# louislung/DAE_RNN_News_Recommendation

Hardware: NVIDIA H100
Metric: articles/sec (higher is better)
Workload: dtype f32

## Files before the change

### dae_rnn_news_recommendation_b200/_cabi.py

```python
import ctypes
import ctypes as C
import os
from pathlib import Path

_PKG = Path(__file__).resolve().parent
LIB_PATH = Path(os.environ.get('DAE_SM100_LIB', _PKG / 'libdae_sm100.so'))

ACT = {'none': 0, 'sigmoid': 1, 'tanh': 2}
LOSS = {'cross_entropy': 0, 'mean_squared': 1, 'cosine_proximity': 2}
STRATEGY = {'none': 0, 'batch_all': 1, 'batch_hard': 2, 'explicit': 3}
OPT = {'gradient_descent': 0, 'ada_grad': 1, 'momentum': 2, 'adam': 3}
STAT = {'cost': 0, 'ae_loss': 1, 'triplet_loss': 2, 'fraction': 3, 'num': 4, 'sum_w': 5, 'n_valid': 6, 'sum_lw': 7,
        'triplet_sum': 8, 'n_active': 9}
STAT_SLOTS = 16
MAX_TRIPLET_BATCH = 32768
MAX_BLOCKED_BATCH = 262144


def act_code(name):
    return ACT.get(name, 0)


p, i32, i64, f32, u64, sz = C.c_void_p, C.c_int32, C.c_int64, C.c_float, C.c_uint64, C.c_size_t

_SIGNATURES = {
    'dae_version': (C.c_int, []),
    'dae_last_error': (C.c_int, [C.c_char_p, sz]),
    'dae_batch_prepare': (C.c_int, [p, i64, p, i32, p, i32, p, p, p, p, p, p, p]),
    'dae_batch_prepare_next': (C.c_int, [p, i64, i64, p, i32, p, i32, p, p, p, p, p, p, p]),
    'dae_batch_prepare_blocked': (C.c_int, [p, i64, p, i32, p, i32, p, p, p, p, p, p, p]),
    'dae_batch_prepare_next_blocked': (C.c_int, [p, i64, i64, p, i32, p, i32, p, p, p, p, p, p, p]),
    'dae_batch_commit': (C.c_int, [i32, p, p, p, p, p, p, p, p, p, p, p, p, p]),
    'dae_batch_prepare_explicit': (C.c_int, [p, i64, p, i32, i64, p, p, p]),
    'dae_step_advance': (C.c_int, [p, i64, p]),
    'dae_encode_csr_fwd': (C.c_int, [p, p, p, p, i32, i32, i32, f32, p, p, i32, p, i64, p, p, p, i64, p]),
    'dae_encode_csr_fwd_hot': (C.c_int, [p, p, p, i32, i32, i32, f32, p, p, i32, p, i64, p, p, i32, i32, p]),
    'dae_col_scan': (C.c_int, [p, i32, p, p, p]),
    'dae_encode_csr_bwd_gather': (C.c_int, [p, p, p, p, i32, i32, i32, f32, p, p, i32, p, p, i64, p, p, i32, p, p, p, p, p, p, p]),
    'dae_encode_csr_bwd': (C.c_int, [p, p, p, p, i32, i32, i32, f32, p, p, i32, p, p, i64, p, p, i32, p]),
    'dae_sgemm': (C.c_int, [i32, i32, i32, f32, p, i64, i64, p, i64, i64, f32, p, i64, p]),
    'dae_split_bf16': (C.c_int, [p, i32, i32, i64, p, p, i64, i32, f32, p]),
    'dae_sym_split_bf16': (C.c_int, [p, i32, i64, f32, p, p, i64, p]),
    'dae_gemm_bf16x3': (C.c_int, [i32, i32, i32, f32, p, p, i64, i32, p, p, i64, i32, p, i64, i32, i32, p, i32, i32, p]),
    'dae_gemm_config': (C.c_int, [i32, i32]),
    'dae_decode_prepare': (C.c_int, [i32, i32, p, p, p, p, p, p]),
    'dae_decode_fused_bf16x3': (C.c_int, [i32, i32, i32, p, p, i64, p, p, i64, p, p, p, p, p, i32, i32, p, p, p, p, i64, p, p, i32, p]),
    'dae_reduce_parts': (C.c_int, [p, i32, i32, p, p]),
    'dae_decode_loss_bwd': (C.c_int, [p, p, p, p, i32, i32, p, i32, i32, p, p, p, i64, p, p]),
    'dae_colsum': (C.c_int, [p, i32, i32, i64, p, p]),
    'dae_triplet_batch_all': (C.c_int, [p, i64, i32, p, p, p, i64, p, i32, p, p, i64, p]),
    'dae_triplet_config': (C.c_int, [i32]),
    'dae_gemm_sym_bf16x3': (C.c_int, [i32, i32, f32, p, p, i64, p, p, i64, p, i64, i32, p]),
    'dae_triplet_batch_hard': (C.c_int, [p, i64, i32, p, p, i64, p, p, p]),
    'dae_triplet_batch_all_rows': (C.c_int, [p, i64, i32, i32, i32, p, p, p, i64, p, i32, p, p, i64, p]),
    'dae_triplet_batch_hard_rows': (C.c_int, [p, i64, i32, i32, i32, p, p, i64, p, p, p]),
    'dae_triplet_batch_hard_finish': (C.c_int, [p, i32, p, p, i32, i64, p]),
    'dae_triplet_explicit': (C.c_int, [p, p, p, i32, i32, i64, f32, p, p, p, p, p]),
    'dae_step_finalize': (C.c_int, [p, p, i32, p, i32, i32, f32, p, p, p, p]),
    'dae_optimizer_step': (C.c_int, [p, p, p, p, i64, i32, f32, f32, f32, i32, p, p, p, i32, i32, i64, p]),
    'dae_rownorm_split_bf16': (C.c_int, [p, i32, i32, i64, i32, p, p, i64, p, i64, p]),
    'dae_row_argmax': (C.c_int, [p, i32, i32, i64, i64, i32, p, p, p]),
    'dae_similarity_topk_bf16x3': (C.c_int, [i32, i32, i32, p, p, i64, p, p, i64, i32, i64, i32, i32, p, i64, p, p, p]),
    'dae_similarity_topk_workspace': (C.c_int, [i32, i32, i32, i32, p]),
    'dae_csr_similarity_topk': (C.c_int, [p, p, p, i32, i64, i32, p, p, p, i32, i64, i32, i32, i64, i32, i32, p, i64, p, p, p]),
    'dae_csr_similarity_topk_workspace': (C.c_int, [i32, i32, i64, i32, i32, i32, p]),
    'dae_similarity_topk_excl_bf16x3': (C.c_int, [i32, i32, i32, p, p, i64, p, p, i64, i32, i64, i32, i32, p, i64, p, p, p, p, i64, p]),
    'dae_csr_similarity_topk_excl': (C.c_int, [p, p, p, i32, i64, i32, p, p, p, i32, i64, i32, i32, i64, i32, i32, p, i64, p, p, p, p,
                                               i64, p]),
    'dae_similarity_topk_groups_bf16x3': (C.c_int, [i32, i32, i32, p, p, i64, p, p, i64, i32, i64, i32, i32, p, i64, p, p, p, p, i64, p,
                                                    p]),
    'dae_csr_similarity_topk_groups': (C.c_int, [p, p, p, i32, i64, i32, p, p, p, i32, i64, i32, i32, i64, i32, i32, p, i64, p, p, p, p,
# ... 121 lines not shown
```

### dae_rnn_news_recommendation_b200/csrc/encode.cu

```cuda
#include <algorithm>
#include <cstdlib>
#include <cuda_bf16.h>
#include "common.cuh"

namespace dae {

template <int VW> struct Vec;
template <> struct Vec<4> { using T = float4; };
template <> struct Vec<2> { using T = float2; };
template <> struct Vec<1> { using T = float; };

template <int VW>
__device__ __forceinline__ void ldg_vec(const float* p, float (&out)[VW]) {
  if constexpr (VW == 4) { const float4 v = __ldg(reinterpret_cast<const float4*>(p)); out[0] = v.x; out[1] = v.y; out[2] = v.z; out[3] = v.w; }
  else if constexpr (VW == 2) { const float2 v = __ldg(reinterpret_cast<const float2*>(p)); out[0] = v.x; out[1] = v.y; }
  else { out[0] = __ldg(p); }
}

constexpr int kEncThreads = 128;

template <int NT = 128>
__device__ __forceinline__ int stage_row_chunk(const int32_t* __restrict__ indices, const float* __restrict__ values,
                                               int64_t base, int64_t p1, float in_scale, int* s_col, float* s_val,
                                               int* s_wcnt) {
// ... 260 lines not shown
  if (tid == 0) s_carry = 0;
  __syncthreads();
  for (int base = 0; base < F; base += kChunkElems) {
    const int n = min(kChunkElems, F - base);
    for (int i = tid; i < kChunkElems; i += 1024) s[i] = (i < n) ? col_count[base + i] : 0;
    __syncthreads();
    int v[kPer], sum = 0;
#pragma unroll
    for (int j = 0; j < kPer; ++j) { v[j] = s[tid * kPer + j]; sum += v[j]; }
    int incl = sum;
#pragma unroll
    for (int o = 1; o < 32; o <<= 1) { const int t = __shfl_up_sync(0xffffffffu, incl, o); if (lane >= o) incl += t; }
    if (lane == 31) s_warp[wid] = incl;
    __syncthreads();
    if (wid == 0) {
      int w = s_warp[lane], wi = w;
#pragma unroll
      for (int o = 1; o < 32; o <<= 1) { const int t = __shfl_up_sync(0xffffffffu, wi, o); if (lane >= o) wi += t; }
      s_warp[lane] = wi - w;
    }
    __syncthreads();
    int run = s_carry + s_warp[wid] + incl - sum;
#pragma unroll
    for (int j = 0; j < kPer; ++j) { s[tid * kPer + j] = run; run += v[j]; }
    __syncthreads();
    for (int i = tid; i < n; i += 1024) { const int x = s[i]; col_start[base + i] = x; col_cursor[base + i] = x; }
    __syncthreads();
    if (tid == 1023) s_carry = run;
    __syncthreads();
  }
  if (tid == 0) col_start[F] = s_carry;
}

constexpr int kRowsPerCta = 4;

template <int ACT, bool DET = false>
__global__ void __launch_bounds__(32 * kRowsPerCta) encode_bwd_rows_kernel(
    const int64_t* __restrict__ indptr, const int32_t* __restrict__ indices, const float* __restrict__ values,
    const int32_t* __restrict__ rows, int n_rows, int H, float in_scale, const float* __restrict__ E, const float* __restrict__ bh,
    float* __restrict__ dE, const float* __restrict__ dE_add, int64_t ldE, float* __restrict__ dbh, int32_t* __restrict__ col_cursor, int32_t* __restrict__ ent_col,
    int32_t* __restrict__ ent_row, float* __restrict__ ent_val) {
  extern __shared__ float s_part[];
  const int tid = threadIdx.x, warp = tid >> 5, lane = tid & 31;
  const int r = blockIdx.x * kRowsPerCta + warp;
  float* part = s_part + (int64_t)warp * H;
  if (r < n_rows) {
    for (int h = lane; h < H; h += 32) {
      const float fb = act_fwd<ACT>(__ldg(bh + h));
      const float fa = E[(int64_t)r * ldE + h] + fb;
      const float de = dE[(int64_t)r * ldE + h] + (dE_add ? dE_add[(int64_t)r * ldE + h] : 0.0f);
      const float da = de * act_grad_from_y<ACT>(fa);
      dE[(int64_t)r * ldE + h] = da;
      part[h] = da - act_grad_from_y<ACT>(fb) * de;
    }
  } else {
    for (int h = lane; h < H; h += 32) part[h] = 0.0f;
  }
  __syncthreads();
  for (int h = tid; h < H; h += 32 * kRowsPerCta) {
    float t = 0.0f;
#pragma unroll
    for (int w = 0; w < kRowsPerCta; ++w) t += s_part[(int64_t)w * H + h];
    if constexpr (DET) dbh[(int64_t)blockIdx.x * H + h] = t;
    else atomicAdd(dbh + h, t);
  }
  if constexpr (DET) return;
  if (r < n_rows) {
    const int64_t row = rows ? (int64_t)rows[r] : (int64_t)r;
    const int64_t p0 = indptr[row], p1 = indptr[row + 1];
    for (int64_t p = p0 + lane; p < p1; p += 32) {
      const float v = __ldg(values + p) * in_scale;
      if (v != 0.0f) {
        const int col = __ldg(indices + p);
        const int slot = atomicAdd(col_cursor + col, 1);
        ent_col[slot] = col;
        ent_row[slot] = r;
        ent_val[slot] = v;
      }
    }
  }
}

constexpr int kChunk = 32;

template <int VW, int NC>
__global__ void __launch_bounds__(kEncThreads) encode_bwd_gather_kernel(const int32_t* __restrict__ col_start, int F,
                                                                        const int32_t* __restrict__ ent_col,
                                                                        const int32_t* __restrict__ ent_row,
                                                                        const float* __restrict__ ent_val, int H,
                                                                        const float* __restrict__ dA, int64_t ldE,
                                                                        float* __restrict__ dW) {
  __shared__ int s_c[kChunk];
  __shared__ int s_r[kChunk];
  __shared__ float s_v[kChunk];
  const int tid = threadIdx.x;
  const int total = col_start[F];
  int hcol[NC];
#pragma unroll
  for (int c = 0; c < NC; ++c) hcol[c] = (tid + c * kEncThreads) * VW;

  for (int base = blockIdx.x * kChunk; base < total; base += gridDim.x * kChunk) {
    const int n = min(kChunk, total - base);
    __syncthreads();
    if (tid < n) { s_c[tid] = ent_col[base + tid]; s_r[tid] = ent_row[base + tid]; s_v[tid] = ent_val[base + tid]; }
    __syncthreads();
    float acc[NC][VW];
#pragma unroll
    for (int c = 0; c < NC; ++c)
#pragma unroll
      for (int k = 0; k < VW; ++k) acc[c][k] = 0.0f;
    int cur = s_c[0];
    for (int q0 = 0; q0 < n; q0 += 8) {
// ... 301 lines not shown
extern "C" int dae_encode_csr_fwd_groups(const int64_t* indptr, const int32_t* indices, const float* values, const int32_t* rows,
                                         int32_t n_rows, int32_t F, int32_t H, float in_scale, const float* W, const float* bh,
                                         int32_t enc_act, float* E, int64_t ldE, int32_t* col_count, void* e_hi, void* e_lo,
                                         int64_t ld_split, int32_t groups, void* stream) {
  using namespace dae;
  DAE_REQUIRE(groups == 1 || groups == 4, "dae_encode_csr_fwd_groups: groups = %d, 1 or 4", groups);
  return encode_fwd("dae_encode_csr_fwd_groups", indptr, indices, values, rows, n_rows, F, H, in_scale, W, bh, enc_act, E, ldE, col_count,
                    e_hi, e_lo, ld_split, groups, stream);
}

extern "C" int dae_encode_csr_bwd(const int64_t* indptr, const int32_t* indices, const float* values, const int32_t* rows,
                                  int32_t n_rows, int32_t F, int32_t H, float in_scale, const float* E, const float* bh,
                                  int32_t enc_act, float* dE, const float* dE_add, int64_t ldE, float* dW, float* dbh, int32_t dbh_zeroed,
                                  void* stream) {
  using namespace dae;
  DAE_REQUIRE(indptr && indices && values && E && bh && dE && dW && dbh, "dae_encode_csr_bwd: null pointer");
  DAE_REQUIRE(n_rows >= 0 && F > 0 && H > 0 && ldE >= H, "dae_encode_csr_bwd: bad shape");
  cudaStream_t st = (cudaStream_t)stream;
  if (!dbh_zeroed) DAE_CUDA(cudaMemsetAsync(dbh, 0, sizeof(float) * H, st));
  if (n_rows == 0) return DAE_OK;
  const int vw = pick_vw(H, H, dW);
  const int nc = pick_nc(H, vw);
  if (nc < 0) { set_error("dae_encode_csr_bwd: H=%d too large", H); return DAE_ERR_UNSUPPORTED; }
  dim3 grid(n_rows);
  DAE_DISPATCH_ACT(enc_act, ACT, {
    if (vw == 4) launch_bwd_nc<ACT, 4>(nc, grid, st, indptr, indices, values, rows, H, in_scale, E, bh, dE, dE_add, ldE, dW, dbh);
    else if (vw == 2) launch_bwd_nc<ACT, 2>(nc, grid, st, indptr, indices, values, rows, H, in_scale, E, bh, dE, dE_add, ldE, dW, dbh);
    else launch_bwd_nc<ACT, 1>(nc, grid, st, indptr, indices, values, rows, H, in_scale, E, bh, dE, dE_add, ldE, dW, dbh);
  });
  DAE_CHECK_LAUNCH("dae_encode_csr_bwd");
  return DAE_OK;
}

extern "C" int dae_encode_csr_bwd_gather(const int64_t* indptr, const int32_t* indices, const float* values, const int32_t* rows,
                                         int32_t n_rows, int32_t F, int32_t H, float in_scale, const float* E, const float* bh,
                                         int32_t enc_act, float* dE, const float* dE_add, int64_t ldE, float* dW, float* dbh,
                                         int32_t dbh_zeroed, const int32_t* col_count, int32_t* col_start, int32_t* col_cursor,
                                         int32_t* ent_col, int32_t* ent_row, float* ent_val, void* stream) {
  using namespace dae;
  DAE_REQUIRE(indptr && indices && values && E && bh && dE && dW && dbh && col_start && col_cursor && ent_col && ent_row && ent_val,
              "dae_encode_csr_bwd_gather: null pointer");
  DAE_REQUIRE(n_rows >= 0 && F > 0 && H > 0 && ldE >= H, "dae_encode_csr_bwd_gather: bad shape");
  cudaStream_t st = (cudaStream_t)stream;
  if (!dbh_zeroed) DAE_CUDA(cudaMemsetAsync(dbh, 0, sizeof(float) * H, st));
  if (n_rows == 0) return DAE_OK;
  int vw = pick_vw(H, ldE, dE);
  if (pick_vw(H, H, dW) < vw) vw = pick_vw(H, H, dW);
  const int nc = pick_nc(H, vw);
  if (nc < 0 || nc > 2) { set_error("dae_encode_csr_bwd_gather: H=%d not supported (use dae_encode_csr_bwd)", H); return DAE_ERR_UNSUPPORTED; }
  if (col_count) col_scan_kernel<<<1, 1024, 0, st>>>(col_count, F, col_start, col_cursor);
  DAE_DISPATCH_ACT(enc_act, ACT, {
    encode_bwd_rows_kernel<ACT><<<(n_rows + kRowsPerCta - 1) / kRowsPerCta, 32 * kRowsPerCta, sizeof(float) * kRowsPerCta * H, st>>>(indptr, indices, values, rows, n_rows, H, in_scale, E, bh, dE, dE_add, ldE, dbh, col_cursor,
                                                               ent_col, ent_row, ent_val);
  });
#define DAE_GATHER(VW, NC) encode_bwd_gather_kernel<VW, NC><<<sm_count() * 16, kEncThreads, 0, st>>>(col_start, F, ent_col, ent_row, ent_val, H, dE, ldE, dW)
#define DAE_GATHER_NC(VW) \
  do { if (nc == 1) DAE_GATHER(VW, 1); else DAE_GATHER(VW, 2); } while (0)
  if (vw == 4) DAE_GATHER_NC(4); else if (vw == 2) DAE_GATHER_NC(2); else DAE_GATHER_NC(1);
#undef DAE_GATHER_NC
#undef DAE_GATHER
  DAE_CHECK_LAUNCH("dae_encode_csr_bwd_gather");
  return DAE_OK;
}

extern "C" int dae_col_scan(const int32_t* col_count, int32_t F, int32_t* col_start, int32_t* col_cursor, void* stream) {
  using namespace dae;
  DAE_REQUIRE(col_count && col_start && col_cursor && F > 0, "dae_col_scan: bad arguments");
  col_scan_kernel<<<1, 1024, 0, (cudaStream_t)stream>>>(col_count, F, col_start, col_cursor);
  DAE_CHECK_LAUNCH("dae_col_scan");
  return DAE_OK;
}

extern "C" int dae_encode_csr_fwd_hot(const int64_t* indptr, const int32_t* indices, const float* values, int32_t n_rows, int32_t F,
                                      int32_t H, float in_scale, const float* W, const float* bh, int32_t enc_act, float* E, int64_t ldE,
                                      const int32_t* hot_cols, const int32_t* hot_slot, int32_t K, int32_t groups, void* stream) {
  using namespace dae;
  DAE_REQUIRE(indptr && indices && values && W && bh && E && hot_cols && hot_slot, "dae_encode_csr_fwd_hot: null pointer");
  DAE_REQUIRE(n_rows >= 0 && F > 0 && H > 0 && ldE >= H && K >= 1, "dae_encode_csr_fwd_hot: bad shape");
  DAE_REQUIRE(H % 4 == 0 && ldE % 4 == 0 && ((uintptr_t)W & 15) == 0 && ((uintptr_t)E & 15) == 0 && H <= 8 * kEncThreads,
              "dae_encode_csr_fwd_hot: needs H %% 4 == 0, H <= 1024 and 16-byte aligned W / E (use dae_encode_csr_fwd otherwise)");
  const size_t smem = (size_t)K * H * 4;
  DAE_REQUIRE(smem <= 200 * 1024, "dae_encode_csr_fwd_hot: K * H * 4 = %zu bytes of staged rows exceed 200 KB", smem);
  if (n_rows == 0) return DAE_OK;
  cudaStream_t st = (cudaStream_t)stream;
  const int sms = sm_count();
  const int nc = (H + 4 * kEncThreads - 1) / (4 * kEncThreads);
  const int G = (groups >= 8) ? 8 : 4;
  int per_sm = (int)((220 * 1024) / (smem + 8 * 1024));
  if (per_sm < 1) per_sm = 1;
  if (per_sm * G * kEncThreads > 2048) per_sm = 2048 / (G * kEncThreads);
  const int want = (n_rows + G - 1) / G;
  const int grid = want < sms * per_sm ? want : sms * per_sm;
#define DAE_HOT(ACT, NC, GG)                                                                                                       \
  do {                                                                                                                            \
// ... 15 lines not shown
  DAE_REQUIRE(bytes && n_rows >= 1 && F > 0 && H > 0 && cap_nnz >= 0, "dae_encode_csr_bwd_det_workspace: bad arguments");
  *bytes = det_layout(n_rows, F, H, cap_nnz).bytes;
  return DAE_OK;
}

extern "C" int dae_encode_csr_bwd_det(const int64_t* indptr, const int32_t* indices, const float* values, const int32_t* rows,
                                      int32_t n_rows, int32_t F, int32_t H, float in_scale, const float* E, const float* bh,
                                      int32_t enc_act, float* dE, const float* dE_add, int64_t ldE, float* dbh, const int32_t* col_count,
                                      int64_t cap_nnz, void* workspace, int64_t workspace_bytes, void* stream) {
  using namespace dae;
  DAE_REQUIRE(indptr && indices && values && E && bh && dE && dbh && col_count && workspace, "dae_encode_csr_bwd_det: null pointer");
  DAE_REQUIRE(n_rows >= 1 && F > 0 && H > 0 && ldE >= H && cap_nnz >= 0, "dae_encode_csr_bwd_det: bad shape");
  const DetLayout L = det_layout(n_rows, F, H, cap_nnz);
  DAE_REQUIRE(workspace_bytes >= L.bytes, "dae_encode_csr_bwd_det: workspace of %lld bytes, need %lld", (long long)workspace_bytes,
              (long long)L.bytes);
  const size_t smem = sizeof(float) * kRowsPerCta * H;
  DAE_REQUIRE(smem <= 200 * 1024, "dae_encode_csr_bwd_det: H=%d too large", H);
  cudaStream_t st = (cudaStream_t)stream;
  uint8_t* w = (uint8_t*)workspace;
  int32_t* col_start = (int32_t*)(w + L.off_start);
  int32_t* tile = (int32_t*)(w + L.off_tile);
  int32_t* ent_col = (int32_t*)(w + L.off_col);
  int32_t* ent_row = (int32_t*)(w + L.off_row);
  float* ent_val = (float*)(w + L.off_val);
  float* dbh_part = (float*)(w + L.off_dbh);
  col_scan_kernel<<<1, 1024, 0, st>>>(col_count, F, col_start, (int32_t*)(w + L.off_cursor));
  DAE_CUDA(cudaMemsetAsync(tile, 0, sizeof(int32_t) * (size_t)L.T * F, st));
  det_tile_count_kernel<<<(n_rows + 7) / 8, 256, 0, st>>>(indptr, indices, values, rows, n_rows, F, L.RT, in_scale, tile);
  det_tile_scan_kernel<<<(F + 255) / 256, 256, 0, st>>>(tile, L.T, F, col_start);
  det_place_kernel<<<(L.T + 3) / 4, 128, 0, st>>>(indptr, indices, values, rows, n_rows, F, L.RT, L.T, in_scale, tile, ent_col, ent_row, ent_val);
  DAE_DISPATCH_ACT(enc_act, ACT, {
    auto kern = encode_bwd_rows_kernel<ACT, true>;
    if (smem > 48 * 1024) DAE_CUDA(cudaFuncSetAttribute(kern, cudaFuncAttributeMaxDynamicSharedMemorySize, (int)smem));
    kern<<<(unsigned)L.n_cta, 32 * kRowsPerCta, smem, st>>>(indptr, indices, values, rows, n_rows, H, in_scale, E, bh, dE, dE_add, ldE,
                                                            dbh_part, nullptr, nullptr, nullptr, nullptr);
  });
  float* dbh_group = (float*)(w + L.off_dbh2);
  det_group_sum_kernel<<<dim3((H + 127) / 128, (unsigned)L.n_groups), 128, 0, st>>>(dbh_part, (int)L.n_cta, H, dbh_group);
  int rc = dae_reduce_parts(dbh_group, (int32_t)L.n_groups, H, dbh, stream);
  if (rc) return rc;
  const int vw = (H % 4 == 0 && ldE % 4 == 0 && ((uintptr_t)dE & 15) == 0) ? 4 : ((H % 2 == 0 && ldE % 2 == 0 && ((uintptr_t)dE & 7) == 0) ? 2 : 1);
  const int64_t want = L.n_chunks;
  const int grid = (int)std::min<int64_t>(want, (int64_t)sm_count() * 16);
  float* colsum = (float*)(w + L.off_colsum);
  float* parts = (float*)(w + L.off_parts);
  if (vw == 4) encode_bwd_gather_det_kernel<4><<<grid, kEncThreads, 0, st>>>(col_start, F, ent_col, ent_row, ent_val, H, dE, ldE, L.CH, colsum, parts);
  else if (vw == 2) encode_bwd_gather_det_kernel<2><<<grid, kEncThreads, 0, st>>>(col_start, F, ent_col, ent_row, ent_val, H, dE, ldE, L.CH, colsum, parts);
  else encode_bwd_gather_det_kernel<1><<<grid, kEncThreads, 0, st>>>(col_start, F, ent_col, ent_row, ent_val, H, dE, ldE, L.CH, colsum, parts);
  DAE_CHECK_LAUNCH("dae_encode_csr_bwd_det");
  return DAE_OK;
}

extern "C" int dae_encode_sparse_dw_add(int32_t n_rows, int32_t F, int32_t H, int64_t cap_nnz, const void* workspace, int64_t workspace_bytes,
                                        float* dW, void* stream) {
  using namespace dae;
  DAE_REQUIRE(workspace && dW && n_rows >= 1 && F > 0 && H > 0 && cap_nnz >= 0, "dae_encode_sparse_dw_add: bad arguments");
  const DetLayout L = det_layout(n_rows, F, H, cap_nnz);
  DAE_REQUIRE(workspace_bytes >= L.bytes, "dae_encode_sparse_dw_add: workspace of %lld bytes, need %lld", (long long)workspace_bytes,
              (long long)L.bytes);
  const uint8_t* w = (const uint8_t*)workspace;
  encode_sparse_dw_add_kernel<<<std::min(F, 65535), 128, 0, (cudaStream_t)stream>>>((const int32_t*)(w + L.off_start), F, H, L.CH,
                                                                                   (const float*)(w + L.off_colsum),
                                                                                   (const float*)(w + L.off_parts), dW);
  DAE_CHECK_LAUNCH("dae_encode_sparse_dw_add");
  return DAE_OK;
}
```

### dae_rnn_news_recommendation_b200/engine.py

```python
import ctypes
import os

import numpy as np
import scipy.sparse as sp
import torch

from . import _cabi
from ._cabi import call, ptr, STAT, STAT_SLOTS

_BATCH_ALL, _BATCH_HARD, _EXPLICIT = (_cabi.STRATEGY[k] for k in ('batch_all', 'batch_hard', 'explicit'))
_COSINE = _cabi.LOSS['cosine_proximity']


def _stream():
    return torch.cuda.current_stream().cuda_stream


def canonical_csr(x):
    if isinstance(x, np.ndarray):
        m = sp.csr_matrix(x)
    else:
        m = sp.csr_matrix(x)
    if not m.has_canonical_format:
        m = m.copy()
# ... 671 lines not shown
                with torch.cuda.stream(sideB):
                    self._k('dae_col_scan', ptr(self.col_count), F, ptr(self.col_start), ptr(self.col_cursor), sideB.cuda_stream)
                    ev_scan = self._record(sideB)
        if stage_fork:
            self._fork(main, sideA)
            with torch.cuda.stream(sideA):
                self._stage_next_batch(*stage_next, B, sideA)
        if tc:
            self._decode_tc(B, weight, train, prepared=dec_prepared)
        else:
            self._decode_and_backward(B, weight, train)
        if not train:
            if explicit_B:
                self._triplet_explicit(explicit_B, main)
            self._finalize(B, weight, stats_log_row, main)
            return
        if branch_a:
            self._fork(main, sideA)
            with torch.cuda.stream(sideA):
                self._finalize(B, weight, stats_log_row, sideA)
        if tc:
            Whl, dZhl = (self.W_hi, self.W_lo), (self.dZ_hi, self.dZ_lo)
            if not branch_b:
                self._dW_gemm(B, accumulate=0)
            det = self.deterministic
            self._tc_gemm(B, H, F, 1.0, dZhl, 0, Whl, 1, self.dE, H, k_splits=-1, accumulate=1 if (branch_b and not det) else 0,
                          tag='gemm_decode_dE', ws=self.gemm_ws[0] if det else None)
        if explicit_B:
            self._triplet_explicit(explicit_B, main)
        if branch_b:
            self._fork(main, sideB)
            with torch.cuda.stream(sideB):
                self._dW_gemm(B, accumulate=1)
        if ev_mined is not None:
            main.wait_event(ev_mined)
        if mines and not tc:
            self._gemm(B, H, B, self.alpha, self.G, B, 1, self.E, 1, H, 1.0, self.dE, H, tag='gemm_dE_tri')
            self._gemm(B, H, B, self.alpha, self.G, 1, B, self.E, 1, H, 1.0, self.dE, H, tag='gemm_dE_tri')
        if branch_b and gather:
            main.wait_event(ev_scan)
        self._encode_backward(B, dE_add=self.dE2 if (tc and mines) else None, dbh_zeroed=1 if branch_b else 0,
                              scan_done=branch_b and gather)
        if not branch_a:
            self._finalize(B, weight, stats_log_row, main)
        elif stage_next is not None:
            with torch.cuda.stream(sideA):
                self._stage_next_batch(*stage_next, B, sideA)
        if branch_b:
            self._fork(sideB, main)
        if self.enc_bwd_mode == 'det':
            self._k('dae_encode_sparse_dw_add', B, F, H, self._ent_cap, ptr(self.enc_det_ws), self.enc_det_ws.numel(), ptr(self._gW()),
                    main.cuda_stream)
        if not defer_update:
            self._apply_update()
        if used_a:
            self._fork(sideA, main)

    def _triplet(self, name, *args, stream, anchors=0, n_launch=1):
        if not self.deterministic:
            self._k(name, *args, stream, n_launch=n_launch)
            return
        self._k(name + '_det', *args, ptr(self.loss_slots), stream, n_launch=n_launch)
        self._sum_loss_slots(anchors, stream)

    def _sum_loss_slots(self, anchors, stream):
        if self.deterministic and anchors:
            self._k('dae_triplet_loss_sum', ptr(self.loss_slots), anchors, ptr(self.stats), stream)

    def _triplet_explicit(self, Bx, stream):
        E, d, H = self.E, self.dE, self.H
        self._triplet('dae_triplet_explicit', ptr(E[0:Bx]), ptr(E[Bx:2 * Bx]), ptr(E[2 * Bx:3 * Bx]), Bx, H, H, self.alpha, ptr(d[0:Bx]),
                      ptr(d[Bx:2 * Bx]), ptr(d[2 * Bx:3 * Bx]), ptr(self.stats), stream=stream.cuda_stream, anchors=Bx)

    def _dE_triplet(self, B, stream):
        st = stream.cuda_stream
# ... 87 lines not shown
            return self.read_stats()
        finally:
            self.csr, self.csr_c, self.values_c, self.labels, self.in_scale = saved

    def _decode_and_backward(self, B, weight, train=True):
        F, H, st = self.F, self.H, _stream()
        c, rows = self.csr, self.rows
        self._gemm(B, F, H, 1.0, self.E, H, 1, self.W, H, 1, 0.0, self.Z, F, tag='gemm_decode_fwd')
        self._k('dae_decode_loss_bwd', ptr(c.indptr), ptr(c.indices), ptr(c.values), ptr(rows), B, F, ptr(self.bv),
                self.dec_act, self.loss, ptr(weight), ptr(self.stats), ptr(self.Z), F, ptr(self.row_loss), st)
        if not train:
            return
        self._k('dae_colsum', ptr(self.Z), B, F, F, ptr(self._gbv()), st)
        self._gemm(F, H, B, 1.0, self.Z, 1, F, self.E, 1, H, 0.0, self._gW(), H, tag='gemm_decode_dW')
        self._gemm(B, H, F, 1.0, self.Z, F, 1, self.W, 1, H, 0.0, self.dE, H, tag='gemm_decode_dE')

    def _decode_tc(self, B, weight, train=True, prepared=0):
        F, H, st = self.F, self.H, _stream()
        c, rows = self.csr, self.rows
        Ehl, Whl = (self.E_hi, self.E_lo), (self.W_hi, self.W_lo)
        if self.loss != _COSINE:
            det = self.deterministic
            self._k('dae_decode_fused_bf16x3_det' if det else 'dae_decode_fused_bf16x3', B, F, H, ptr(self.E_hi), ptr(self.E_lo), self.Hp, ptr(self.W_hi), ptr(self.W_lo),
                    self.Hp, ptr(c.indptr), ptr(c.indices), ptr(c.values), ptr(rows), ptr(self.bv), self.dec_act, self.loss,
                    ptr(weight), ptr(self.stats), ptr(self.dZ_hi), ptr(self.dZ_lo), self.Fp, ptr(self.loss_parts if det else self.row_loss),
                    ptr(self.tile_ptr), int(prepared), st, n_launch=1 if prepared else 2, tag='gemm_decode_fwd')
        else:
            self._tc_gemm(B, F, H, 1.0, Ehl, 0, Whl, 0, self.Z, F, tag='gemm_decode_fwd')
            self._k('dae_decode_loss_bwd', ptr(c.indptr), ptr(c.indices), ptr(c.values), ptr(rows), B, F, ptr(self.bv),
                    self.dec_act, self.loss, ptr(weight), ptr(self.stats), ptr(self.Z), F, ptr(self.row_loss), st)
            if train:
                self._tc_split(self.Z, B, F, F, self.dZ_hi, self.dZ_lo)

    def _encode_backward(self, B, dE_add=None, dbh_zeroed=0, scan_done=False):
        F, H, st = self.F, self.H, _stream()
        c = self.csr_c
        head = (ptr(c.indptr), ptr(c.indices), ptr(self.values_c), ptr(self.rows), B, F, H, self.in_scale, ptr(self.E), ptr(self.bh),
                self.enc_act, ptr(self.dE), ptr(dE_add), H)
        if self.enc_bwd_mode == 'det':
            self._k('dae_encode_csr_bwd_det', *head, ptr(self._gbh()), ptr(self.col_count), self._ent_cap, ptr(self.enc_det_ws),
                    self.enc_det_ws.numel(), st, tag='dae_encode_csr_bwd',
                    n_launch=8)
        elif self.enc_bwd_mode == 'gather':
            self._k('dae_encode_csr_bwd_gather', *head, ptr(self._gW()), ptr(self._gbh()), int(dbh_zeroed), None if scan_done else ptr(self.col_count),
                    ptr(self.col_start), ptr(self.col_cursor), ptr(self.ent_col), ptr(self.ent_row), ptr(self.ent_val), st, n_launch=3,
                    tag='dae_encode_csr_bwd')
        else:
            self._k('dae_encode_csr_bwd', *head, ptr(self._gW()), ptr(self._gbh()), int(dbh_zeroed), st)

    def _setup_multimem(self, n_blocks=132):
        import torch.distributed._symmetric_memory as symm
        group = self.pg if self.pg is not None else torch.distributed.group.WORLD
        grad = symm.empty(self.n_params, dtype=torch.float32, device=self.device)
        grad.zero_()
        h_grad = symm.rendezvous(grad, group)
        if not getattr(h_grad, 'has_multicast_support', False) or not h_grad.multicast_ptr:
            raise _cabi.DaeError('DAE_ALLREDUCE=multimem: this process group has no NVSwitch multicast support')
        flags = symm.empty(2 * n_blocks * self.world, dtype=torch.int32, device=self.device)
        flags.zero_()
        h_flags = symm.rendezvous(flags, group)
        self.grad = grad
        self._mm = {'grad': h_grad, 'flags': h_flags, 'flag_buf': flags, 'mc_ptr': int(h_grad.multicast_ptr),
                    'epochs': torch.zeros(n_blocks, dtype=torch.int32, device=self.device),
                    'flag_ptrs': int(h_flags.buffer_ptrs_dev), 'rank': int(h_grad.rank), 'blocks': int(n_blocks)}
        torch.cuda.synchronize(self.device)
        torch.distributed.barrier(group)

    def _allreduce_grad(self):
        if self.allreduce_mode == 'multimem':
            m = self._mm
            self._k('dae_allreduce_multimem', m['mc_ptr'], m['flag_ptrs'], ptr(m['epochs']), m['rank'], self.world, self.n_params, m['blocks'], _stream())
        else:
            torch.distributed.all_reduce(self.grad, group=self.pg)

    def _apply_update(self, reduce=True):
        F, H, st = self.F, self.H, _stream()
        gscale = 1.0
        if self.world > 1:
# ... 128 lines not shown
```

### include/dae_sm100.h

```cpp
#ifndef DAE_SM100_H
#define DAE_SM100_H

#include <stddef.h>
#include <stdint.h>

#ifdef __cplusplus
extern "C" {
#endif

#define DAE_OK 0
#define DAE_ERR_BAD_ARG (-1)
#define DAE_ERR_CUDA (-2)
#define DAE_ERR_UNSUPPORTED (-3)

#define DAE_ACT_NONE 0
#define DAE_ACT_SIGMOID 1
#define DAE_ACT_TANH 2

#define DAE_LOSS_CE 0
#define DAE_LOSS_MSE 1
#define DAE_LOSS_COSINE 2

#define DAE_TRIPLET_NONE 0
#define DAE_TRIPLET_BATCH_ALL 1
// ... 27 lines not shown
                      int32_t* seg_hi, float* weight_out, double* stats, void* stream);
int dae_batch_prepare_next(const int32_t* perm, int64_t n_perm, int64_t stride, const int64_t* ctl, int32_t B,
                           const float* labels_all, int32_t strategy, int32_t* rows_s, float* labels_s,
                           int32_t* seg_lo_s, int32_t* seg_hi_s, float* weight_s, double* stats_s, void* stream);
int dae_batch_prepare_blocked(const int32_t* perm, int64_t offset, const int64_t* ctl, int32_t B, const float* labels_all,
                              int32_t strategy, int32_t* rows_out, float* labels_out, int32_t* seg_lo,
                              int32_t* seg_hi, float* weight_out, double* stats, void* stream);
int dae_batch_prepare_next_blocked(const int32_t* perm, int64_t n_perm, int64_t stride, const int64_t* ctl, int32_t B,
                                   const float* labels_all, int32_t strategy, int32_t* rows_s, float* labels_s,
                                   int32_t* seg_lo_s, int32_t* seg_hi_s, float* weight_s, double* stats_s, void* stream);
int dae_batch_commit(int32_t B, const int32_t* rows_s, const float* labels_s, const int32_t* seg_lo_s,
                     const int32_t* seg_hi_s, const float* weight_s, const double* stats_s, int32_t* rows,
                     float* labels_b, int32_t* seg_lo, int32_t* seg_hi, float* weight, double* stats, void* stream);
int dae_batch_prepare_explicit(const int32_t* perm, int64_t offset, const int64_t* ctl, int32_t B, int64_t n_each,
                               int32_t* rows_out, double* stats, void* stream);

int dae_encode_csr_fwd(const int64_t* indptr, const int32_t* indices, const float* values,
                       const int32_t* rows, int32_t n_rows, int32_t F, int32_t H, float in_scale,
                       const float* W, const float* bh, int32_t enc_act, float* E, int64_t ldE,
                       int32_t* col_count, void* e_hi, void* e_lo, int64_t ld_split, void* stream);

int dae_encode_csr_bwd(const int64_t* indptr, const int32_t* indices, const float* values,
                       const int32_t* rows, int32_t n_rows, int32_t F, int32_t H, float in_scale,
                       const float* E, const float* bh, int32_t enc_act, float* dE, const float* dE_add,
                       int64_t ldE, float* dW, float* dbh, int32_t dbh_zeroed, void* stream);

int dae_col_scan(const int32_t* col_count, int32_t F, int32_t* col_start, int32_t* col_cursor, void* stream);
int dae_encode_csr_bwd_gather(const int64_t* indptr, const int32_t* indices, const float* values,
                              const int32_t* rows, int32_t n_rows, int32_t F, int32_t H, float in_scale,
                              const float* E, const float* bh, int32_t enc_act, float* dE, const float* dE_add,
                              int64_t ldE, float* dW, float* dbh, int32_t dbh_zeroed, const int32_t* col_count,
                              int32_t* col_start, int32_t* col_cursor, int32_t* ent_col, int32_t* ent_row,
                              float* ent_val, void* stream);

int dae_encode_csr_fwd_hot(const int64_t* indptr, const int32_t* indices, const float* values, int32_t n_rows,
                           int32_t F, int32_t H, float in_scale, const float* W, const float* bh, int32_t enc_act,
                           float* E, int64_t ldE, const int32_t* hot_cols, const int32_t* hot_slot, int32_t K,
                           int32_t groups, void* stream);

int dae_sgemm(int32_t M, int32_t N, int32_t K, float alpha, const float* A, int64_t sam, int64_t sak,
              const float* B, int64_t sbn, int64_t sbk, float beta, float* C, int64_t ldc, void* stream);

int dae_split_bf16(const float* src, int32_t rows, int32_t cols, int64_t ld_src, void* hi, void* lo,
                   int64_t ld_dst, int32_t ones_col, float scale, void* stream);
int dae_sym_split_bf16(const float* G, int32_t B, int64_t ldg, float alpha, void* hi, void* lo, int64_t ld,
                       void* stream);
int dae_gemm_bf16x3(int32_t M, int32_t N, int32_t K, float alpha, const void* a_hi, const void* a_lo,
                    int64_t lda, int32_t a_mn_major, const void* b_hi, const void* b_lo, int64_t ldb,
                    int32_t b_mn_major, float* C, int64_t ldc, int32_t n_store, int32_t special_col,
                    float* special_out, int32_t k_splits, int32_t accumulate, void* stream);
int dae_gemm_sym_bf16x3(int32_t M, int32_t N, float alpha, const void* g_hi, const void* g_lo, int64_t ldg,
                        const void* b_hi, const void* b_lo, int64_t ldb, float* C, int64_t ldc, int32_t accumulate,
                        void* stream);
int dae_gemm_config(int32_t pair_mode, int32_t lean);
int dae_decode_prepare(int32_t Brows, int32_t F, const int64_t* indptr, const int32_t* indices, const int32_t* rows,
                       float* row_loss_part, int32_t* tile_ptr, void* stream);
int dae_decode_fused_bf16x3(int32_t Brows, int32_t F, int32_t K, const void* e_hi, const void* e_lo,
                            int64_t lde, const void* w_hi, const void* w_lo, int64_t ldw,
                            const int64_t* indptr, const int32_t* indices, const float* values,
                            const int32_t* rows, const float* bv, int32_t dec_act, int32_t loss_func,
                            const float* weight, const double* stats, void* dz_hi, void* dz_lo,
                            int64_t ld_dz, float* row_loss_part, int32_t* tile_ptr, int32_t prepared, void* stream);
int dae_reduce_parts(const float* parts, int32_t n_parts, int32_t n, float* out, void* stream);

int dae_decode_loss_bwd(const int64_t* indptr, const int32_t* indices, const float* values,
                        const int32_t* rows, int32_t n_rows, int32_t F, const float* bv, int32_t dec_act,
// ... 269 lines not shown
```

Measured before the change: 2.289 million.

## Split CSR bucketing out of encoder backward and schedule it before triplet wait

The CSR entry bucketing (per-column atomic slot assignment) moves out of the encoder backward rows kernel into its own kernel. The engine launches it on the main stream right after the column scan, before waiting on triplet mining. This overlaps bucketing with side-stream work and leaves the rows kernel with only the activation gradient. It costs one extra kernel launch, and the bucket pass reads the CSR in a separate kernel instead of reusing the rows kernel's warps.

```diff
diff --git a/dae_rnn_news_recommendation_b200/_cabi.py b/dae_rnn_news_recommendation_b200/_cabi.py
--- a/dae_rnn_news_recommendation_b200/_cabi.py
+++ b/dae_rnn_news_recommendation_b200/_cabi.py
@@ -37,6 +37,8 @@
     'dae_encode_csr_fwd_hot': (C.c_int, [p, p, p, i32, i32, i32, f32, p, p, i32, p, i64, p, p, i32, i32, p]),
     'dae_col_scan': (C.c_int, [p, i32, p, p, p]),
     'dae_encode_csr_bwd_gather': (C.c_int, [p, p, p, p, i32, i32, i32, f32, p, p, i32, p, p, i64, p, p, i32, p, p, p, p, p, p, p]),
+    'dae_encode_bucket': (C.c_int, [p, p, p, p, i32, f32, p, p, p, p, p]),
+    'dae_encode_csr_bwd_placed': (C.c_int, [i32, i32, i32, p, p, i32, p, p, i64, p, p, i32, p, p, p, p, p]),
     'dae_encode_csr_bwd': (C.c_int, [p, p, p, p, i32, i32, i32, f32, p, p, i32, p, p, i64, p, p, i32, p]),
     'dae_sgemm': (C.c_int, [i32, i32, i32, f32, p, i64, i64, p, i64, i64, f32, p, i64, p]),
     'dae_split_bf16': (C.c_int, [p, i32, i32, i64, p, p, i64, i32, f32, p]),
diff --git a/dae_rnn_news_recommendation_b200/csrc/encode.cu b/dae_rnn_news_recommendation_b200/csrc/encode.cu
--- a/dae_rnn_news_recommendation_b200/csrc/encode.cu
+++ b/dae_rnn_news_recommendation_b200/csrc/encode.cu
@@ -316,14 +316,34 @@
   if (tid == 0) col_start[F] = s_carry;
 }
 
+constexpr int kBucketRowsPerCta = 8;
+
+__global__ void __launch_bounds__(32 * kBucketRowsPerCta) encode_bucket_kernel(
+    const int64_t* __restrict__ indptr, const int32_t* __restrict__ indices, const float* __restrict__ values,
+    const int32_t* __restrict__ rows, int n_rows, float in_scale, int32_t* __restrict__ col_cursor, int32_t* __restrict__ ent_col,
+    int32_t* __restrict__ ent_row, float* __restrict__ ent_val) {
+  const int r = blockIdx.x * kBucketRowsPerCta + (threadIdx.x >> 5), lane = threadIdx.x & 31;
+  if (r >= n_rows) return;
+  const int64_t row = rows ? (int64_t)rows[r] : (int64_t)r;
+  const int64_t p0 = indptr[row], p1 = indptr[row + 1];
+  for (int64_t p = p0 + lane; p < p1; p += 32) {
+    const float v = __ldg(values + p) * in_scale;
+    if (v != 0.0f) {
+      const int col = __ldg(indices + p);
+      const int slot = atomicAdd(col_cursor + col, 1);
+      ent_col[slot] = col;
+      ent_row[slot] = r;
+      ent_val[slot] = v;
+    }
+  }
+}
+
 constexpr int kRowsPerCta = 4;
 
 template <int ACT, bool DET = false>
 __global__ void __launch_bounds__(32 * kRowsPerCta) encode_bwd_rows_kernel(
-    const int64_t* __restrict__ indptr, const int32_t* __restrict__ indices, const float* __restrict__ values,
-    const int32_t* __restrict__ rows, int n_rows, int H, float in_scale, const float* __restrict__ E, const float* __restrict__ bh,
-    float* __restrict__ dE, const float* __restrict__ dE_add, int64_t ldE, float* __restrict__ dbh, int32_t* __restrict__ col_cursor, int32_t* __restrict__ ent_col,
-    int32_t* __restrict__ ent_row, float* __restrict__ ent_val) {
+    int n_rows, int H, const float* __restrict__ E, const float* __restrict__ bh, float* __restrict__ dE, const float* __restrict__ dE_add,
+    int64_t ldE, float* __restrict__ dbh) {
   extern __shared__ float s_part[];
   const int tid = threadIdx.x, warp = tid >> 5, lane = tid & 31;
   const int r = blockIdx.x * kRowsPerCta + warp;
@@ -347,21 +367,6 @@
     for (int w = 0; w < kRowsPerCta; ++w) t += s_part[(int64_t)w * H + h];
     if constexpr (DET) dbh[(int64_t)blockIdx.x * H + h] = t;
     else atomicAdd(dbh + h, t);
-  }
-  if constexpr (DET) return;
-  if (r < n_rows) {
-    const int64_t row = rows ? (int64_t)rows[r] : (int64_t)r;
-    const int64_t p0 = indptr[row], p1 = indptr[row + 1];
-    for (int64_t p = p0 + lane; p < p1; p += 32) {
-      const float v = __ldg(values + p) * in_scale;
-      if (v != 0.0f) {
-        const int col = __ldg(indices + p);
-        const int slot = atomicAdd(col_cursor + col, 1);
-        ent_col[slot] = col;
-        ent_row[slot] = r;
-        ent_val[slot] = v;
-      }
-    }
   }
 }
 
@@ -729,6 +734,41 @@
   return DAE_OK;
 }
 
+namespace dae {
+
+static void launch_gather(int vw, int nc, const int32_t* col_start, int F, const int32_t* ent_col, const int32_t* ent_row,
+                          const float* ent_val, int H, const float* dA, int64_t ldE, float* dW, cudaStream_t st) {
+#define DAE_GATHER(VW, NC) encode_bwd_gather_kernel<VW, NC><<<sm_count() * 16, kEncThreads, 0, st>>>(col_start, F, ent_col, ent_row, ent_val, H, dA, ldE, dW)
+#define DAE_GATHER_NC(VW) \
+  do { if (nc == 1) DAE_GATHER(VW, 1); else DAE_GATHER(VW, 2); } while (0)
+  if (vw == 4) DAE_GATHER_NC(4); else if (vw == 2) DAE_GATHER_NC(2); else DAE_GATHER_NC(1);
+#undef DAE_GATHER_NC
+#undef DAE_GATHER
+}
+
+static void launch_bucket(const int64_t* indptr, const int32_t* indices, const float* values, const int32_t* rows, int n_rows,
+                          float in_scale, int32_t* col_cursor, int32_t* ent_col, int32_t* ent_row, float* ent_val, cudaStream_t st) {
+  encode_bucket_kernel<<<(n_rows + kBucketRowsPerCta - 1) / kBucketRowsPerCta, 32 * kBucketRowsPerCta, 0, st>>>(
+      indptr, indices, values, rows, n_rows, in_scale, col_cursor, ent_col, ent_row, ent_val);
+}
+
+static int encode_bwd_placed(const char* name, int32_t n_rows, int32_t F, int32_t H, const float* E, const float* bh, int32_t enc_act,
+                             float* dE, const float* dE_add, int64_t ldE, float* dW, float* dbh, const int32_t* col_start,
+                             const int32_t* ent_col, const int32_t* ent_row, const float* ent_val, cudaStream_t st) {
+  int vw = pick_vw(H, ldE, dE);
+  if (pick_vw(H, H, dW) < vw) vw = pick_vw(H, H, dW);
+  const int nc = pick_nc(H, vw);
+  if (nc < 0 || nc > 2) { set_error("%s: H=%d not supported (use dae_encode_csr_bwd)", name, H); return DAE_ERR_UNSUPPORTED; }
+  DAE_DISPATCH_ACT(enc_act, ACT, {
+    encode_bwd_rows_kernel<ACT><<<(n_rows + kRowsPerCta - 1) / kRowsPerCta, 32 * kRowsPerCta, sizeof(float) * kRowsPerCta * H, st>>>(
+        n_rows, H, E, bh, dE, dE_add, ldE, dbh);
+  });
+  launch_gather(vw, nc, col_start, F, ent_col, ent_row, ent_val, H, dE, ldE, dW, st);
+  return DAE_OK;
+}
+
+}
+
 extern "C" int dae_encode_csr_bwd_gather(const int64_t* indptr, const int32_t* indices, const float* values, const int32_t* rows,
                                          int32_t n_rows, int32_t F, int32_t H, float in_scale, const float* E, const float* bh,
                                          int32_t enc_act, float* dE, const float* dE_add, int64_t ldE, float* dW, float* dbh,
@@ -746,17 +786,38 @@
   const int nc = pick_nc(H, vw);
   if (nc < 0 || nc > 2) { set_error("dae_encode_csr_bwd_gather: H=%d not supported (use dae_encode_csr_bwd)", H); return DAE_ERR_UNSUPPORTED; }
   if (col_count) col_scan_kernel<<<1, 1024, 0, st>>>(col_count, F, col_start, col_cursor);
-  DAE_DISPATCH_ACT(enc_act, ACT, {
-    encode_bwd_rows_kernel<ACT><<<(n_rows + kRowsPerCta - 1) / kRowsPerCta, 32 * kRowsPerCta, sizeof(float) * kRowsPerCta * H, st>>>(indptr, indices, values, rows, n_rows, H, in_scale, E, bh, dE, dE_add, ldE, dbh, col_cursor,
-                                                               ent_col, ent_row, ent_val);
-  });
-#define DAE_GATHER(VW, NC) encode_bwd_gather_kernel<VW, NC><<<sm_count() * 16, kEncThreads, 0, st>>>(col_start, F, ent_col, ent_row, ent_val, H, dE, ldE, dW)
-#define DAE_GATHER_NC(VW) \
-  do { if (nc == 1) DAE_GATHER(VW, 1); else DAE_GATHER(VW, 2); } while (0)
-  if (vw == 4) DAE_GATHER_NC(4); else if (vw == 2) DAE_GATHER_NC(2); else DAE_GATHER_NC(1);
-#undef DAE_GATHER_NC
-#undef DAE_GATHER
+  launch_bucket(indptr, indices, values, rows, n_rows, in_scale, col_cursor, ent_col, ent_row, ent_val, st);
+  const int rc = encode_bwd_placed("dae_encode_csr_bwd_gather", n_rows, F, H, E, bh, enc_act, dE, dE_add, ldE, dW, dbh, col_start, ent_col,
+                                   ent_row, ent_val, st);
+  if (rc) return rc;
   DAE_CHECK_LAUNCH("dae_encode_csr_bwd_gather");
+  return DAE_OK;
+}
+
+extern "C" int dae_encode_bucket(const int64_t* indptr, const int32_t* indices, const float* values, const int32_t* rows, int32_t n_rows,
+                                 float in_scale, int32_t* col_cursor, int32_t* ent_col, int32_t* ent_row, float* ent_val, void* stream) {
+  using namespace dae;
+  DAE_REQUIRE(indptr && indices && values && col_cursor && ent_col && ent_row && ent_val && n_rows >= 0, "dae_encode_bucket: bad arguments");
+  if (n_rows == 0) return DAE_OK;
+  launch_bucket(indptr, indices, values, rows, n_rows, in_scale, col_cursor, ent_col, ent_row, ent_val, (cudaStream_t)stream);
+  DAE_CHECK_LAUNCH("dae_encode_bucket");
+  return DAE_OK;
+}
+
+extern "C" int dae_encode_csr_bwd_placed(int32_t n_rows, int32_t F, int32_t H, const float* E, const float* bh, int32_t enc_act, float* dE,
+                                         const float* dE_add, int64_t ldE, float* dW, float* dbh, int32_t dbh_zeroed,
+                                         const int32_t* col_start, const int32_t* ent_col, const int32_t* ent_row, const float* ent_val,
+                                         void* stream) {
+  using namespace dae;
+  DAE_REQUIRE(E && bh && dE && dW && dbh && col_start && ent_col && ent_row && ent_val, "dae_encode_csr_bwd_placed: null pointer");
+  DAE_REQUIRE(n_rows >= 0 && F > 0 && H > 0 && ldE >= H, "dae_encode_csr_bwd_placed: bad shape");
+  cudaStream_t st = (cudaStream_t)stream;
+  if (!dbh_zeroed) DAE_CUDA(cudaMemsetAsync(dbh, 0, sizeof(float) * H, st));
+  if (n_rows == 0) return DAE_OK;
+  const int rc = encode_bwd_placed("dae_encode_csr_bwd_placed", n_rows, F, H, E, bh, enc_act, dE, dE_add, ldE, dW, dbh, col_start, ent_col,
+                                   ent_row, ent_val, st);
+  if (rc) return rc;
+  DAE_CHECK_LAUNCH("dae_encode_csr_bwd_placed");
   return DAE_OK;
 }
 
@@ -838,8 +899,7 @@
   DAE_DISPATCH_ACT(enc_act, ACT, {
     auto kern = encode_bwd_rows_kernel<ACT, true>;
     if (smem > 48 * 1024) DAE_CUDA(cudaFuncSetAttribute(kern, cudaFuncAttributeMaxDynamicSharedMemorySize, (int)smem));
-    kern<<<(unsigned)L.n_cta, 32 * kRowsPerCta, smem, st>>>(indptr, indices, values, rows, n_rows, H, in_scale, E, bh, dE, dE_add, ldE,
-                                                            dbh_part, nullptr, nullptr, nullptr, nullptr);
+    kern<<<(unsigned)L.n_cta, 32 * kRowsPerCta, smem, st>>>(n_rows, H, E, bh, dE, dE_add, ldE, dbh_part);
   });
   float* dbh_group = (float*)(w + L.off_dbh2);
   det_group_sum_kernel<<<dim3((H + 127) / 128, (unsigned)L.n_groups), 128, 0, st>>>(dbh_part, (int)L.n_cta, H, dbh_group);
diff --git a/dae_rnn_news_recommendation_b200/engine.py b/dae_rnn_news_recommendation_b200/engine.py
--- a/dae_rnn_news_recommendation_b200/engine.py
+++ b/dae_rnn_news_recommendation_b200/engine.py
@@ -727,15 +727,18 @@
             self._fork(main, sideB)
             with torch.cuda.stream(sideB):
                 self._dW_gemm(B, accumulate=1)
+        if branch_b and gather:
+            main.wait_event(ev_scan)
+            c = self.csr_c
+            self._k('dae_encode_bucket', ptr(c.indptr), ptr(c.indices), ptr(self.values_c), ptr(self.rows), B, self.in_scale,
+                    ptr(self.col_cursor), ptr(self.ent_col), ptr(self.ent_row), ptr(self.ent_val), main.cuda_stream)
         if ev_mined is not None:
             main.wait_event(ev_mined)
         if mines and not tc:
             self._gemm(B, H, B, self.alpha, self.G, B, 1, self.E, 1, H, 1.0, self.dE, H, tag='gemm_dE_tri')
             self._gemm(B, H, B, self.alpha, self.G, 1, B, self.E, 1, H, 1.0, self.dE, H, tag='gemm_dE_tri')
-        if branch_b and gather:
-            main.wait_event(ev_scan)
         self._encode_backward(B, dE_add=self.dE2 if (tc and mines) else None, dbh_zeroed=1 if branch_b else 0,
-                              scan_done=branch_b and gather)
+                              placed=branch_b and gather)
         if not branch_a:
             self._finalize(B, weight, stats_log_row, main)
         elif stage_next is not None:
@@ -889,7 +892,7 @@
             if train:
                 self._tc_split(self.Z, B, F, F, self.dZ_hi, self.dZ_lo)
 
-    def _encode_backward(self, B, dE_add=None, dbh_zeroed=0, scan_done=False):
+    def _encode_backward(self, B, dE_add=None, dbh_zeroed=0, placed=False):
         F, H, st = self.F, self.H, _stream()
         c = self.csr_c
         head = (ptr(c.indptr), ptr(c.indices), ptr(self.values_c), ptr(self.rows), B, F, H, self.in_scale, ptr(self.E), ptr(self.bh),
@@ -898,9 +901,13 @@
             self._k('dae_encode_csr_bwd_det', *head, ptr(self._gbh()), ptr(self.col_count), self._ent_cap, ptr(self.enc_det_ws),
                     self.enc_det_ws.numel(), st, tag='dae_encode_csr_bwd',
                     n_launch=8)
+        elif placed:
+            self._k('dae_encode_csr_bwd_placed', B, F, H, ptr(self.E), ptr(self.bh), self.enc_act, ptr(self.dE), ptr(dE_add), H,
+                    ptr(self._gW()), ptr(self._gbh()), int(dbh_zeroed), ptr(self.col_start), ptr(self.ent_col), ptr(self.ent_row),
+                    ptr(self.ent_val), st, n_launch=2, tag='dae_encode_csr_bwd')
         elif self.enc_bwd_mode == 'gather':
-            self._k('dae_encode_csr_bwd_gather', *head, ptr(self._gW()), ptr(self._gbh()), int(dbh_zeroed), None if scan_done else ptr(self.col_count),
-                    ptr(self.col_start), ptr(self.col_cursor), ptr(self.ent_col), ptr(self.ent_row), ptr(self.ent_val), st, n_launch=3,
+            self._k('dae_encode_csr_bwd_gather', *head, ptr(self._gW()), ptr(self._gbh()), int(dbh_zeroed), ptr(self.col_count),
+                    ptr(self.col_start), ptr(self.col_cursor), ptr(self.ent_col), ptr(self.ent_row), ptr(self.ent_val), st, n_launch=4,
                     tag='dae_encode_csr_bwd')
         else:
             self._k('dae_encode_csr_bwd', *head, ptr(self._gW()), ptr(self._gbh()), int(dbh_zeroed), st)
diff --git a/include/dae_sm100.h b/include/dae_sm100.h
--- a/include/dae_sm100.h
+++ b/include/dae_sm100.h
@@ -83,6 +83,13 @@
                               int64_t ldE, float* dW, float* dbh, int32_t dbh_zeroed, const int32_t* col_count,
                               int32_t* col_start, int32_t* col_cursor, int32_t* ent_col, int32_t* ent_row,
                               float* ent_val, void* stream);
+int dae_encode_bucket(const int64_t* indptr, const int32_t* indices, const float* values, const int32_t* rows,
+                      int32_t n_rows, float in_scale, int32_t* col_cursor, int32_t* ent_col, int32_t* ent_row,
+                      float* ent_val, void* stream);
+int dae_encode_csr_bwd_placed(int32_t n_rows, int32_t F, int32_t H, const float* E, const float* bh, int32_t enc_act,
+                              float* dE, const float* dE_add, int64_t ldE, float* dW, float* dbh, int32_t dbh_zeroed,
+                              const int32_t* col_start, const int32_t* ent_col, const int32_t* ent_row,
+                              const float* ent_val, void* stream);
 
 int dae_encode_csr_fwd_hot(const int64_t* indptr, const int32_t* indices, const float* values, int32_t n_rows,
                            int32_t F, int32_t H, float in_scale, const float* W, const float* bh, int32_t enc_act,
```

New measurement: 2.253 million, median of 6. -1.6%, worse.
